# Sbte/RAILS

Hardware: AMD Instinct MI355X
Metric: RAILS iterations/sec (+ A*V SpMM HBM GB/s in roofline), m=1M rows/GPU, k=128, fp64 (higher is better)
Workload: dtype f64

## Files before the change

### include/rails_hip.h

```cpp
#ifndef RAILS_HIP_H
#define RAILS_HIP_H

#include <stddef.h>
#include <stdint.h>

#ifdef __cplusplus
extern "C" {
#endif

#define RAILS_OK 0
#define RAILS_EINVAL -1
#define RAILS_EHIP -2
#define RAILS_ENOMEM -3
#define RAILS_ELAPACK -4
#define RAILS_ECOMM -5
#define RAILS_ENODEV -6

typedef struct rails_ctx rails_ctx;
typedef struct rails_csr rails_csr;
typedef struct rails_panel rails_panel;

const char *rails_last_error(void);
const char *rails_version(void);


int rails_ctx_create(int device, void *stream, rails_ctx **out);
int rails_ctx_destroy(rails_ctx *ctx);
int rails_ctx_sync(rails_ctx *ctx);
void *rails_ctx_stream(rails_ctx *ctx);
int rails_ctx_stats(rails_ctx *ctx, char *buf, int cap);
int rails_ctx_set_meter(rails_ctx *ctx, int on);

int rails_ctx_set_seed(rails_ctx *ctx, uint64_t seed, uint64_t first_stream);
int rails_ctx_rng_state(rails_ctx *ctx, uint64_t *seed, uint64_t *next_stream);

int rails_ctx_set_partition(rails_ctx *ctx, int rank, int nranks, int64_t row0, int64_t m_global);

typedef int (*rails_allreduce_fn)(void *user, double *dev_buf, size_t n, void *stream);
int rails_ctx_set_allreduce(rails_ctx *ctx, rails_allreduce_fn fn, void *user);

#define RAILS_RCCL_ID_BYTES 128
int rails_rccl_unique_id(void *id_out);
int rails_ctx_init_rccl(rails_ctx *ctx, const void *id, int nranks, int rank);
int rails_ctx_set_rccl(rails_ctx *ctx, void *nccl_comm);
int rails_ctx_rccl_size(const rails_ctx *ctx);

typedef int (*rails_halo_fn)(void *user, const double *send_buf, double *recv_buf, int ncols, void *stream);


int rails_csr_create(rails_ctx *ctx, int64_t m_local, int64_t n_cols_ext, const int64_t *rowptr,
                     const int32_t *col, const double *val, rails_csr **out);
typedef int (*rails_apply_fn)(void *user, int trans, const rails_panel *X, int xc0, int nc, rails_panel *Y, int yc0);
int rails_csr_create_callback(rails_ctx *ctx, int64_t m_local, rails_apply_fn fn, void *user, rails_csr **out);
int rails_csr_destroy(rails_csr *A);
int64_t rails_csr_rows(const rails_csr *A);
int64_t rails_csr_nnz(const rails_csr *A);

int rails_csr_set_halo(rails_csr *A, int64_t n_send, const int64_t *send_rows, int64_t n_ghost,
                       rails_halo_fn fn, void *user);

int rails_csr_set_halo_counts(rails_csr *A, int nranks, const int64_t *send_counts, const int64_t *recv_counts);

int rails_spmm(rails_ctx *ctx, rails_csr *A, int trans, const rails_panel *X, int xc0, int nc,
               rails_panel *Y, int yc0);

int rails_csr_set_variant(rails_csr *A, int variant);
int rails_csr_prepare(rails_ctx *ctx, rails_csr *A, int trans, int nc, int *kernel_ready);
int rails_csr_sweep_stats(rails_csr *A, int nc, double *out);
int rails_csr_create_rect(rails_ctx *ctx, int64_t n_rows, int64_t n_cols, const int64_t *rowptr, const int32_t *col, const double *val,
                          rails_csr **out);
const char *rails_csr_last_kernel(const rails_csr *A);

typedef struct rails_sptrsv rails_sptrsv;
int rails_sptrsv_create(rails_ctx *ctx, int64_t n, const int64_t *rowptr, const int32_t *col, const double *val, int lower, int unit_diag,
                        rails_sptrsv **out);
void rails_sptrsv_destroy(rails_sptrsv *T);
int64_t rails_sptrsv_levels(const rails_sptrsv *T);
int rails_sptrsv_solve(rails_ctx *ctx, const rails_sptrsv *T, rails_panel *X, int c0, int nc);
int rails_panel_permute_rows(rails_ctx *ctx, const rails_panel *X, int xc0, int nc, const int32_t *perm_dev, int scatter, rails_panel *Y, int yc0);
int rails_index_upload(rails_ctx *ctx, const int32_t *host, int64_t n, int32_t **out_dev);
void rails_index_free(rails_ctx *ctx, int32_t *dev);

typedef struct rails_lu rails_lu;
int rails_lu_create(rails_ctx *ctx, int64_t n, const int64_t *L_rowptr, const int32_t *L_col, const double *L_val, const int64_t *U_rowptr,
                    const int32_t *U_col, const double *U_val, const int32_t *perm_r, const int32_t *perm_c, const int32_t *rows, int64_t m_sub,
                    rails_lu **out);
void rails_lu_destroy(rails_lu *lu);
int rails_lu_solve(rails_ctx *ctx, rails_lu *lu, int trans, const rails_panel *X, int xc0, int nc, rails_panel *Y, int yc0);
int rails_lu_stats(const rails_lu *lu, int64_t *info, int cap);
int rails_csr_create_lu(rails_ctx *ctx, rails_lu *lu, rails_csr **out);

typedef struct rails_sweep_plan rails_sweep_plan;
int rails_sweep_plan_create(int64_t m, int64_t ncols, const int64_t *rowptr, const int32_t *col, const double *val,
                            const int *params, rails_sweep_plan **out);
int rails_sweep_plan_destroy(rails_sweep_plan *plan);
int rails_sweep_plan_info(const rails_sweep_plan *plan, int64_t *iinfo, double *dinfo);
int rails_sweep_plan_array(const rails_sweep_plan *plan, int which, const void **ptr, int64_t *count);


int rails_panel_create(rails_ctx *ctx, int64_t m_local, int capacity, rails_panel **out);
int rails_panel_destroy(rails_panel *P);
int64_t rails_panel_rows(const rails_panel *P);
int rails_panel_capacity(const rails_panel *P);
int rails_panel_ld(const rails_panel *P);
void *rails_panel_device_ptr(const rails_panel *P);
int rails_panel_reserve(rails_ctx *ctx, rails_panel *P, int capacity);

int rails_panel_upload(rails_ctx *ctx, rails_panel *P, int c0, int nc, const double *host, int64_t ldh);
int rails_panel_download(rails_ctx *ctx, const rails_panel *P, int c0, int nc, double *host, int64_t ldh);

int rails_panel_fill(rails_ctx *ctx, rails_panel *P, int c0, int nc, double value);
int rails_panel_scale(rails_ctx *ctx, rails_panel *P, int c0, int nc, double s);
int rails_panel_copy(rails_ctx *ctx, const rails_panel *X, int xc0, int nc, rails_panel *Y, int yc0);
int rails_panel_axpy(rails_ctx *ctx, double alpha, const rails_panel *X, int xc0, int nc, rails_panel *Y,
                     int yc0);
int rails_panel_random(rails_ctx *ctx, rails_panel *P, int c0, int nc);

int rails_gram(rails_ctx *ctx, const rails_panel *X, int xc0, int a, const rails_panel *Y, int yc0, int b,
               double *C_host, int ldc);

int rails_panel_gemm(rails_ctx *ctx, double alpha, const rails_panel *X, int xc0, int k, const double *C_host,
                     int ldc, int r, double beta, rails_panel *Y, int yc0);

int rails_ctx_enable_library_gemm(rails_ctx *ctx);
int rails_ctx_library_gemm_ready(const rails_ctx *ctx);

int rails_deferred_reserve(rails_ctx *ctx, int nslots, int64_t doubles_per_slot);
int rails_gram_deferred(rails_ctx *ctx, const rails_panel *X, int xc0, int a, const rails_panel *Y, int yc0, int b, int slot);
int rails_panel_gemm_deferred(rails_ctx *ctx, double alpha, const rails_panel *X, int xc0, int k, int slot, int ld, int r, double beta,
                              rails_panel *Y, int yc0);
int rails_chol_inverse_deferred(rails_ctx *ctx, int slot_in, int w, int slot_out);
int rails_update_gram_deferred(rails_ctx *ctx, double alpha, const rails_panel *X, int xc0, int k, const double *C_host, int ldc, int r,
                               rails_panel *Y, int yc0, int r2, int slot);
int rails_deferred_fetch(rails_ctx *ctx, int slot, int64_t n, double *host_out);

int rails_panel_gemm_wide(rails_ctx *ctx, double alpha, const rails_panel *X, int xc0, int k, const double *C_host, int ldc, int r,
                          double beta, rails_panel *Y, int yc0);

int rails_orthogonalize(rails_ctx *ctx, rails_panel *V, int k_old, int w, int method, int *used);
int rails_orthogonalize_deflated(rails_ctx *ctx, rails_panel *V, int k_old, int w, const rails_panel *N, int nc0, int q, int method, int *used);

int rails_resid_lanczos(rails_ctx *ctx, const rails_panel *AV, int avc0, const rails_panel *MV, int mvc0, int k,
                        const double *T_host, int ldt, const rails_panel *B, int bc0, int p, int L,
                        double *H_host, int ldh, int *steps);

int rails_lanczos_start(rails_ctx *ctx, const rails_panel *AV, int avc0, const rails_panel *MV, int mvc0, int k,
                        const rails_panel *B, int bc0, int p, double *sums_host);

int rails_lanczos_vectors(rails_ctx *ctx, const double *S_host, int lds, int w, rails_panel *Out, int oc0);
int rails_lanczos_last_launch(rails_ctx *ctx, int *nch, int *unroll, int *nblocks);
int rails_lanczos_release(rails_ctx *ctx);

int rails_ctx_reserve_staging(rails_ctx *ctx, size_t bytes);
int rails_timer_start(rails_ctx *ctx);
int rails_timer_stop(rails_ctx *ctx, double *ms);


void rails_sb03md(char dico, char job, char fact, char trans, int n, double *A, int lda, double *X, int ldx,
                  double *scale, int *info);
void rails_sb03md_counts(long *smith, long *schur);
void rails_sb03md_adi_counts(long *extended, long *fresh);
void rails_sb03md_set_pause(int calls);
void rails_dsyev(char jobz, char uplo, int n, double *a, int lda, double *w, int *info);
void rails_dsteqr(char compz, int n, double *d, double *e, double *z, int ldz, double *work, int *info);
void rails_dgemm(char transa, char transb, int m, int n, int k, double alpha, const double *A, int lda, const double *B,
                 int ldb, double beta, double *C, int ldc);
void rails_dtrsm(char side, char uplo, char transa, char diag, int m, int n, double alpha, const double *A, int lda, double *B, int ldb);
void rails_dpotrf(char uplo, int n, double *a, int lda, int *info);
void rails_dpstrf(char uplo, int n, double *a, int lda, int *piv, int *rank, double tol, int *info);
void rails_range_basis(int m, int n, double *a, int lda, double tol, double *q, int ldq, int *rank, int *info);
int rails_host_lapack_init(const char *path);
const char *rails_host_lapack_path(void);

#ifdef __cplusplus
}
#endif
#endif
```

### rails_amd/_lib.py

```python
import ctypes as C
import os

_HERE = os.path.dirname(os.path.abspath(__file__))
LIB_PATH = os.path.join(_HERE, "lib", "librails_hip.so")

_dp = C.POINTER(C.c_double)
_ip = C.POINTER(C.c_int)
_i64p = C.POINTER(C.c_int64)
_i32p = C.POINTER(C.c_int32)
_vp = C.c_void_p

ALLREDUCE_FN = C.CFUNCTYPE(C.c_int, C.c_void_p, C.c_void_p, C.c_size_t, C.c_void_p)
HALO_FN = C.CFUNCTYPE(C.c_int, C.c_void_p, C.c_void_p, C.c_void_p, C.c_int, C.c_void_p)
APPLY_FN = C.CFUNCTYPE(C.c_int, C.c_void_p, C.c_int, C.c_void_p, C.c_int, C.c_int, C.c_void_p, C.c_int)

SIGNATURES = {
    "rails_last_error": (C.c_char_p, []),
    "rails_version": (C.c_char_p, []),
    "rails_ctx_create": (C.c_int, [C.c_int, _vp, C.POINTER(_vp)]),
    "rails_ctx_destroy": (C.c_int, [_vp]),
    "rails_ctx_sync": (C.c_int, [_vp]),
    "rails_ctx_stream": (_vp, [_vp]),
    "rails_ctx_set_meter": (C.c_int, [_vp, C.c_int]),
    "rails_ctx_enable_library_gemm": (C.c_int, [_vp]),
    "rails_ctx_library_gemm_ready": (C.c_int, [_vp]),
    "rails_deferred_reserve": (C.c_int, [_vp, C.c_int, C.c_int64]),
    "rails_gram_deferred": (C.c_int, [_vp, _vp, C.c_int, C.c_int, _vp, C.c_int, C.c_int, C.c_int]),
    "rails_update_gram_deferred": (C.c_int, [_vp, C.c_double, _vp, C.c_int, C.c_int, _dp, C.c_int, C.c_int, _vp, C.c_int, C.c_int, C.c_int]),
    "rails_panel_gemm_deferred": (C.c_int, [_vp, C.c_double, _vp, C.c_int, C.c_int, C.c_int, C.c_int, C.c_int, C.c_double, _vp, C.c_int]),
    "rails_chol_inverse_deferred": (C.c_int, [_vp, C.c_int, C.c_int, C.c_int]),
    "rails_deferred_fetch": (C.c_int, [_vp, C.c_int, C.c_int64, _dp]),
    "rails_ctx_stats": (C.c_int, [_vp, C.c_char_p, C.c_int]),
    "rails_ctx_set_seed": (C.c_int, [_vp, C.c_uint64, C.c_uint64]),
    "rails_ctx_rng_state": (C.c_int, [_vp, C.POINTER(C.c_uint64), C.POINTER(C.c_uint64)]),
    "rails_ctx_set_partition": (C.c_int, [_vp, C.c_int, C.c_int, C.c_int64, C.c_int64]),
    "rails_ctx_set_allreduce": (C.c_int, [_vp, ALLREDUCE_FN, _vp]),
    "rails_rccl_unique_id": (C.c_int, [_vp]),
    "rails_ctx_init_rccl": (C.c_int, [_vp, _vp, C.c_int, C.c_int]),
    "rails_ctx_set_rccl": (C.c_int, [_vp, _vp]),
    "rails_ctx_rccl_size": (C.c_int, [_vp]),
    "rails_csr_set_halo_counts": (C.c_int, [_vp, C.c_int, _i64p, _i64p]),
    "rails_csr_create": (C.c_int, [_vp, C.c_int64, C.c_int64, _i64p, _i32p, _dp, C.POINTER(_vp)]),
    "rails_csr_create_rect": (C.c_int, [_vp, C.c_int64, C.c_int64, _i64p, _i32p, _dp, C.POINTER(_vp)]),
    "rails_csr_create_callback": (C.c_int, [_vp, C.c_int64, APPLY_FN, _vp, C.POINTER(_vp)]),
    "rails_csr_destroy": (C.c_int, [_vp]),
    "rails_csr_rows": (C.c_int64, [_vp]),
    "rails_csr_nnz": (C.c_int64, [_vp]),
    "rails_csr_set_halo": (C.c_int, [_vp, C.c_int64, _i64p, C.c_int64, HALO_FN, _vp]),
    "rails_spmm": (C.c_int, [_vp, _vp, C.c_int, _vp, C.c_int, C.c_int, _vp, C.c_int]),
    "rails_csr_set_variant": (C.c_int, [_vp, C.c_int]),
    "rails_csr_sweep_stats": (C.c_int, [_vp, C.c_int, _dp]),
    "rails_csr_prepare": (C.c_int, [_vp, _vp, C.c_int, C.c_int, C.POINTER(C.c_int)]),
    "rails_csr_last_kernel": (C.c_char_p, [_vp]),
    "rails_sweep_plan_create": (C.c_int, [C.c_int64, C.c_int64, _i64p, _i32p, _dp, _ip, C.POINTER(_vp)]),
    "rails_sweep_plan_destroy": (C.c_int, [_vp]),
    "rails_sweep_plan_info": (C.c_int, [_vp, _i64p, _dp]),
    "rails_sweep_plan_array": (C.c_int, [_vp, C.c_int, C.POINTER(_vp), _i64p]),
    "rails_panel_create": (C.c_int, [_vp, C.c_int64, C.c_int, C.POINTER(_vp)]),
    "rails_panel_destroy": (C.c_int, [_vp]),
    "rails_panel_rows": (C.c_int64, [_vp]),
    "rails_panel_capacity": (C.c_int, [_vp]),
    "rails_panel_ld": (C.c_int, [_vp]),
    "rails_panel_device_ptr": (_vp, [_vp]),
    "rails_panel_reserve": (C.c_int, [_vp, _vp, C.c_int]),
    "rails_panel_upload": (C.c_int, [_vp, _vp, C.c_int, C.c_int, _dp, C.c_int64]),
    "rails_panel_download": (C.c_int, [_vp, _vp, C.c_int, C.c_int, _dp, C.c_int64]),
    "rails_panel_fill": (C.c_int, [_vp, _vp, C.c_int, C.c_int, C.c_double]),
    "rails_panel_scale": (C.c_int, [_vp, _vp, C.c_int, C.c_int, C.c_double]),
    "rails_panel_copy": (C.c_int, [_vp, _vp, C.c_int, C.c_int, _vp, C.c_int]),
    "rails_panel_axpy": (C.c_int, [_vp, C.c_double, _vp, C.c_int, C.c_int, _vp, C.c_int]),
    "rails_sptrsv_create": (C.c_int, [_vp, C.c_int64, _i64p, _i32p, _dp, C.c_int, C.c_int, C.POINTER(_vp)]),
    "rails_sptrsv_destroy": (None, [_vp]),
    "rails_sptrsv_levels": (C.c_int64, [_vp]),
    "rails_sptrsv_solve": (C.c_int, [_vp, _vp, _vp, C.c_int, C.c_int]),
    "rails_panel_permute_rows": (C.c_int, [_vp, _vp, C.c_int, C.c_int, _vp, C.c_int, _vp, C.c_int]),
    "rails_index_upload": (C.c_int, [_vp, _i32p, C.c_int64, C.POINTER(_vp)]),
    "rails_index_free": (None, [_vp, _vp]),
    "rails_lu_create": (C.c_int, [_vp, C.c_int64, _i64p, _i32p, _dp, _i64p, _i32p, _dp, _i32p, _i32p, _i32p, C.c_int64, C.POINTER(_vp)]),
    "rails_lu_destroy": (None, [_vp]),
    "rails_lu_solve": (C.c_int, [_vp, _vp, C.c_int, _vp, C.c_int, C.c_int, _vp, C.c_int]),
    "rails_lu_stats": (C.c_int, [_vp, _i64p, C.c_int]),
    "rails_csr_create_lu": (C.c_int, [_vp, _vp, C.POINTER(_vp)]),
    "rails_panel_random": (C.c_int, [_vp, _vp, C.c_int, C.c_int]),
    "rails_gram": (C.c_int, [_vp, _vp, C.c_int, C.c_int, _vp, C.c_int, C.c_int, _dp, C.c_int]),
    "rails_panel_gemm": (C.c_int, [_vp, C.c_double, _vp, C.c_int, C.c_int, _dp, C.c_int, C.c_int, C.c_double, _vp, C.c_int]),
    "rails_panel_gemm_wide": (C.c_int, [_vp, C.c_double, _vp, C.c_int, C.c_int, _dp, C.c_int, C.c_int, C.c_double, _vp, C.c_int]),
    "rails_orthogonalize": (C.c_int, [_vp, _vp, C.c_int, C.c_int, C.c_int, _ip]),
    "rails_orthogonalize_deflated": (C.c_int, [_vp, _vp, C.c_int, C.c_int, _vp, C.c_int, C.c_int, C.c_int, _ip]),
    "rails_resid_lanczos": (C.c_int, [_vp, _vp, C.c_int, _vp, C.c_int, C.c_int, _dp, C.c_int, _vp, C.c_int, C.c_int, C.c_int,
                                      _dp, C.c_int, _ip]),
    "rails_lanczos_start": (C.c_int, [_vp, _vp, C.c_int, _vp, C.c_int, C.c_int, _vp, C.c_int, C.c_int, _dp]),
    "rails_lanczos_vectors": (C.c_int, [_vp, _dp, C.c_int, C.c_int, _vp, C.c_int]),
    "rails_lanczos_last_launch": (C.c_int, [_vp, _ip, _ip, _ip]),
    "rails_lanczos_release": (C.c_int, [_vp]),
    "rails_timer_start": (C.c_int, [_vp]),
    "rails_timer_stop": (C.c_int, [_vp, _dp]),
    "rails_sb03md": (None, [C.c_char, C.c_char, C.c_char, C.c_char, C.c_int, _dp, C.c_int, _dp, C.c_int, _dp, _ip]),
    "rails_dsyev": (None, [C.c_char, C.c_char, C.c_int, _dp, C.c_int, _dp, _ip]),
    "rails_dsteqr": (None, [C.c_char, C.c_int, _dp, _dp, _dp, C.c_int, _dp, _ip]),
    "rails_ctx_reserve_staging": (C.c_int, [_vp, C.c_size_t]),
    "rails_sb03md_set_pause": (None, [C.c_int]),
    "rails_sb03md_counts": (None, [C.POINTER(C.c_long), C.POINTER(C.c_long)]),
    "rails_sb03md_adi_counts": (None, [C.POINTER(C.c_long), C.POINTER(C.c_long)]),
    "rails_dtrsm": (None, [C.c_char, C.c_char, C.c_char, C.c_char, C.c_int, C.c_int, C.c_double, _dp, C.c_int, _dp, C.c_int]),
    "rails_dgemm": (None, [C.c_char, C.c_char, C.c_int, C.c_int, C.c_int, C.c_double, _dp, C.c_int, _dp, C.c_int, C.c_double, _dp, C.c_int]),
    "rails_dpotrf": (None, [C.c_char, C.c_int, _dp, C.c_int, _ip]),
    "rails_dpstrf": (None, [C.c_char, C.c_int, _dp, C.c_int, _ip, _ip, C.c_double, _ip]),
    "rails_range_basis": (None, [C.c_int, C.c_int, _dp, C.c_int, C.c_double, _dp, C.c_int, _ip, _ip]),
    "rails_host_lapack_init": (C.c_int, [C.c_char_p]),
    "rails_host_lapack_path": (C.c_char_p, []),
}

_lib = None


class RailsError(RuntimeError):
    pass


def load():
    global _lib
    if _lib is not None:
        return _lib
    if not os.path.exists(LIB_PATH):
        raise RailsError(
            "rails_amd: %s is missing -- build it with `python -c 'import __graft_entry__ as g; g.build()'` "
            "or `make -C rails_amd/csrc`; there is no CPU fallback" % LIB_PATH)
    lib = C.CDLL(LIB_PATH, mode=C.RTLD_GLOBAL)
    for name, (res, args) in SIGNATURES.items():
        fn = getattr(lib, name)
        fn.restype = res
        fn.argtypes = args
    try:
        from ._solver_sigs import bind as _bind_solver
        _bind_solver(lib)
    except ImportError:
        pass
    from ._solution_sigs import bind as _bind_solution

    _bind_solution(lib)
    _lib = lib
    return lib


def check(rc, what=""):
    if rc != 0:
        msg = load().rails_last_error()
        raise RailsError("%s failed (code %d): %s" % (what or "rails call", rc, msg.decode() if msg else ""))
```

### rails_amd/csrc/host_numerics.cpp

```cpp
#include <dlfcn.h>

#include <algorithm>
#include <atomic>
#include <chrono>
#include <utility>
#include <cmath>
#include <cstdio>
#include <cstdlib>
#include <cstring>
#include <mutex>
#include <string>
#include <vector>

#include "rails_hip.h"

void rails_set_error(const char *fmt, ...);

namespace {

extern "C" {
typedef int (*lp_select2)(const double *, const double *);
typedef void (*lp_dsyev)(const char *, const char *, const int *, double *, const int *, double *, double *, const int *, int *);
typedef void (*lp_dsyevd)(const char *, const char *, const int *, double *, const int *, double *, double *, const int *, int *, const int *, int *);
typedef void (*lp_dsteqr)(const char *, const int *, double *, double *, double *, const int *, double *, int *);
// ... 106 lines not shown
    return true;
}

void gemm(char ta, char tb, int m, int n, int k, const double *A, int lda, const double *B, int ldb, double *C, int ldc)
{
    const double one = 1.0, zero = 0.0;
    g_lp.dgemm(&ta, &tb, &m, &n, &k, &one, A, &lda, B, &ldb, &zero, C, &ldc);
}

}

extern "C" int rails_host_lapack_init(const char *path)
{
    std::lock_guard<std::mutex> lock(g_lp_mutex);
    if (g_lp.handle) return RAILS_OK;
    if (path && *path && try_open(path)) return RAILS_OK;
    if (const char *env = getenv("RAILS_LAPACK_LIB"))
        if (try_open(env)) return RAILS_OK;
    static const char *dirs[] = {"/usr/local/lib/python3.10/dist-packages/scipy.libs", "/usr/lib/python3/dist-packages/scipy.libs",
                                 nullptr};
    for (int i = 0; dirs[i]; ++i) {
        std::string cmd = std::string("ls ") + dirs[i] + "/libscipy_openblas*.so 2>/dev/null";
        if (FILE *f = popen(cmd.c_str(), "r")) {
            char buf[1024];
            std::vector<std::string> found;
            while (fgets(buf, sizeof(buf), f)) {
                std::string s(buf);
                while (!s.empty() && (s.back() == '\n' || s.back() == ' ')) s.pop_back();
                found.push_back(s);
            }
            pclose(f);
            for (auto &s : found)
                if (try_open(s)) return RAILS_OK;
        }
    }
    static const char *cands[] = {"libopenblas.so.0", "libopenblas.so", "liblapack.so.3", "liblapack.so", "/opt/conda/lib/libmkl_rt.so",
                                  "libmkl_rt.so", nullptr};
    for (int i = 0; cands[i]; ++i)
        if (try_open(cands[i])) return RAILS_OK;
    rails_set_error("no host LAPACK found: set RAILS_LAPACK_LIB to a library exporting dsyev_/dgees_/dtrsyl_/dpotrf_/dgemm_");
    return RAILS_ELAPACK;
}

extern "C" const char *rails_host_lapack_path(void) { return g_lp.path.c_str(); }

static bool all_finite(int rows, int cols, const double *a, int lda)
{
    for (int j = 0; j < cols; ++j)
        for (int i = 0; i < rows; ++i)
            if (!std::isfinite(a[i + (size_t)j * lda])) return false;
    return true;
}

extern "C" void rails_dsyev(char jobz, char uplo, int n, double *a, int lda, double *w, int *info)
{
    if (rails_host_lapack_init(nullptr) != RAILS_OK) {
        *info = -100;
        return;
    }
    if (n <= 0) {
        *info = 0;
        return;
    }
    if (!all_finite(n, n, a, lda)) {
        fprintf(stderr, "rails_dsyev: the matrix holds NaN or Inf entries\n");
        *info = n + 1;
        return;
    }
    if (g_lp.dsyevd && n >= 64 && (jobz == 'V' || jobz == 'v')) {
        int lwork = -1, liwork = -1, iq = 0;
        double wq = 0.0;
        g_lp.dsyevd(&jobz, &uplo, &n, a, &lda, w, &wq, &lwork, &iq, &liwork, info);
        if (*info == 0) {
            lwork = (int)wq + 1;
            liwork = iq + 1;
            std::vector<double> work((size_t)lwork);
            std::vector<int> iwork((size_t)liwork);
            g_lp.dsyevd(&jobz, &uplo, &n, a, &lda, w, work.data(), &lwork, iwork.data(), &liwork, info);
            return;
        }
    }
    int lwork = -1;
    double wq = 0.0;
    g_lp.dsyev(&jobz, &uplo, &n, a, &lda, w, &wq, &lwork, info);
    if (*info) return;
    lwork = (int)wq;
    std::vector<double> work((size_t)std::max(1, lwork));
    g_lp.dsyev(&jobz, &uplo, &n, a, &lda, w, work.data(), &lwork, info);
}

extern "C" void rails_dsteqr(char compz, int n, double *d, double *e, double *z, int ldz, double *work, int *info)
{
    if (rails_host_lapack_init(nullptr) != RAILS_OK) {
        *info = -100;
        return;
    }
    g_lp.dsteqr(&compz, &n, d, e, z, &ldz, work, info);
}

extern "C" void rails_dtrsm(char side, char uplo, char transa, char diag, int m, int n, double alpha, const double *A, int lda, double *B, int ldb)
{
    if (m <= 0 || n <= 0) return;
    const char *force_loops = getenv("RAILS_DTRSM_LOOPS");
    if (!(force_loops && atoi(force_loops) != 0) && rails_host_lapack_init(nullptr) == RAILS_OK && g_lp.dtrsm) {
        g_lp.dtrsm(&side, &uplo, &transa, &diag, &m, &n, &alpha, A, &lda, B, &ldb);
        return;
    }
    const bool left = side == 'L' || side == 'l', upper = uplo == 'U' || uplo == 'u', trans = !(transa == 'N' || transa == 'n'),
               unit = diag == 'U' || diag == 'u';
    const int na = left ? m : n;
    auto a = [&](int i, int j) { return trans ? A[j + (size_t)i * lda] : A[i + (size_t)j * lda]; };
    const bool op_upper = upper != trans;
    for (int j = 0; j < n; ++j)
        for (int i = 0; i < m; ++i) B[i + (size_t)j * ldb] *= alpha;
    if (left) {
        for (int j = 0; j < n; ++j) {
            double *b = B + (size_t)j * ldb;
            if (op_upper)
                for (int i = na - 1; i >= 0; --i) {
                    double s = b[i];
                    for (int l = i + 1; l < na; ++l) s -= a(i, l) * b[l];
                    b[i] = unit ? s : s / a(i, i);
                }
            else
                for (int i = 0; i < na; ++i) {
                    double s = b[i];
                    for (int l = 0; l < i; ++l) s -= a(i, l) * b[l];
                    b[i] = unit ? s : s / a(i, i);
                }
        }
    } else {
        for (int i = 0; i < m; ++i) {
            if (op_upper)
                for (int j = 0; j < na; ++j) {
                    double s = B[i + (size_t)j * ldb];
                    for (int l = 0; l < j; ++l) s -= B[i + (size_t)l * ldb] * a(l, j);
                    B[i + (size_t)j * ldb] = unit ? s : s / a(j, j);
                }
            else
                for (int j = na - 1; j >= 0; --j) {
                    double s = B[i + (size_t)j * ldb];
                    for (int l = j + 1; l < na; ++l) s -= B[i + (size_t)l * ldb] * a(l, j);
                    B[i + (size_t)j * ldb] = unit ? s : s / a(j, j);
                }
        }
    }
}

extern "C" void rails_dgemm(char ta, char tb, int m, int n, int k, double alpha, const double *A, int lda, const double *B, int ldb,
                            double beta, double *C, int ldc)
{
    if (rails_host_lapack_init(nullptr) != RAILS_OK) return;
    g_lp.dgemm(&ta, &tb, &m, &n, &k, &alpha, A, &lda, B, &ldb, &beta, C, &ldc);
}

extern "C" void rails_dpotrf(char uplo, int n, double *a, int lda, int *info)
{
    if (rails_host_lapack_init(nullptr) != RAILS_OK) {
        *info = -100;
        return;
    }
    g_lp.dpotrf(&uplo, &n, a, &lda, info);
}

extern "C" void rails_dpstrf(char uplo, int n, double *a, int lda, int *piv, int *rank, double tol, int *info)
{
    if (rails_host_lapack_init(nullptr) != RAILS_OK) {
        *info = -100;
        return;
    }
    if (g_lp.dpstrf) {
        std::vector<double> work((size_t)2 * (n > 0 ? n : 1));
        g_lp.dpstrf(&uplo, &n, a, &lda, piv, rank, &tol, work.data(), info);
        for (int i = 0; i < n; ++i) piv[i] -= 1;
        return;
    }
    *info = 0;
    if (uplo != 'U' && uplo != 'u') {
        *info = -1;
        return;
    }
    for (int i = 0; i < n; ++i) piv[i] = i;
    int r = 0;
    for (; r < n; ++r) {
        int q = r;
        for (int j = r + 1; j < n; ++j)
            if (a[j + (size_t)j * lda] > a[q + (size_t)q * lda]) q = j;
        if (!(a[q + (size_t)q * lda] > tol)) break;
        if (q != r) {
            std::swap(piv[r], piv[q]);
            std::swap(a[r + (size_t)r * lda], a[q + (size_t)q * lda]);
            for (int i = 0; i < r; ++i) std::swap(a[i + (size_t)r * lda], a[i + (size_t)q * lda]);
            for (int j = q + 1; j < n; ++j) std::swap(a[r + (size_t)j * lda], a[q + (size_t)j * lda]);
            for (int i = r + 1; i < q; ++i) std::swap(a[r + (size_t)i * lda], a[i + (size_t)q * lda]);
        }
        double d = std::sqrt(a[r + (size_t)r * lda]);
        a[r + (size_t)r * lda] = d;
        for (int j = r + 1; j < n; ++j) a[r + (size_t)j * lda] /= d;
        for (int j = r + 1; j < n; ++j) {
            double f = a[r + (size_t)j * lda];
            for (int i = r + 1; i <= j; ++i) a[i + (size_t)j * lda] -= a[r + (size_t)i * lda] * f;
        }
    }
    *rank = r;
    *info = r < n ? 1 : 0;
}

extern "C" void rails_range_basis(int m, int n, double *a, int lda, double tol, double *q, int ldq, int *rank, int *info)
{
    *rank = 0;
    if (rails_host_lapack_init(nullptr) != RAILS_OK || !g_lp.dgeqp3 || !g_lp.dorgqr) {
        *info = -100;
        return;
    }
    if (m <= 0 || n <= 0) {
        *info = 0;
        return;
    }
    const int kmin = m < n ? m : n;
    std::vector<int> jpvt((size_t)n, 0);
    std::vector<double> tau((size_t)kmin);
    double wq = 0.0;
    int lwork = -1;
    g_lp.dgeqp3(&m, &n, a, &lda, jpvt.data(), tau.data(), &wq, &lwork, info);
    if (*info != 0) return;
    lwork = (int)wq + 1;
    std::vector<double> work((size_t)lwork);
    g_lp.dgeqp3(&m, &n, a, &lda, jpvt.data(), tau.data(), work.data(), &lwork, info);
    if (*info != 0) return;
    const double r11 = std::fabs(a[0]);
    int r = 0;
    while (r < kmin && std::fabs(a[r + (size_t)r * lda]) > tol * r11 && r11 > 0.0) ++r;
    *rank = r;
    if (r == 0) return;
    for (int j = 0; j < r; ++j)
        for (int i = 0; i < m; ++i) q[i + (size_t)j * ldq] = a[i + (size_t)j * lda];
    lwork = -1;
    g_lp.dorgqr(&m, &r, &r, q, &ldq, tau.data(), &wq, &lwork, info);
    if (*info != 0) return;
    lwork = (int)wq + 1;
    work.resize((size_t)lwork);
    g_lp.dorgqr(&m, &r, &r, q, &ldq, tau.data(), work.data(), &lwork, info);
}

static int &sb03md_smith_pause()
{
    static thread_local int pause = 0;
    return pause;
}
static int &sb03md_factored_pause()
{
    static thread_local int pause = 0;
    return pause;
}
extern "C" void rails_sb03md_set_pause(int calls) { sb03md_smith_pause() = sb03md_factored_pause() = calls > 0 ? calls : 0; }
static std::atomic<long> g_sb03md_smith{0}, g_sb03md_schur{0};
extern "C" void rails_sb03md_counts(long *smith, long *schur)
{
    if (smith) *smith = g_sb03md_smith.load();
    if (schur) *schur = g_sb03md_schur.load();
}

static bool smith_lyapunov(bool tr, int n, const double *A, int lda, double *X, int ldx)
{
    if (!g_lp.dgetrf || !g_lp.dgetrs) return false;
    const size_t nn = (size_t)n * n;
    std::vector<double> M(nn), S(nn), Ak(nn), Y(nn), T1(nn), T2(nn), C(nn);
    double trace = 0.0;
    for (int j = 0; j < n; ++j) {
        for (int i = 0; i < n; ++i) {
            M[i + (size_t)j * n] = tr ? A[i + (size_t)j * lda] : A[j + (size_t)i * lda];
            C[i + (size_t)j * n] = 0.5 * (X[i + (size_t)j * ldx] + X[j + (size_t)i * ldx]);
        }
        trace += A[j + (size_t)j * lda];
    }
    const double p = -trace / n;
    if (!(p > 0.0) || !std::isfinite(p)) return false;
    S = M;
    for (int j = 0; j < n; ++j) S[j + (size_t)j * n] -= p;
    std::vector<int> ipiv(n);
    int info = 0;
    g_lp.dgetrf(&n, &n, S.data(), &n, ipiv.data(), &info);
    if (info != 0) return false;
    std::fill(Ak.begin(), Ak.end(), 0.0);
    for (int j = 0; j < n; ++j) Ak[j + (size_t)j * n] = 1.0;
    const char N = 'N';
    g_lp.dgetrs(&N, &n, &n, S.data(), &n, ipiv.data(), Ak.data(), &n, &info);
    if (info != 0) return false;
    gemm('N', 'N', n, n, n, Ak.data(), n, C.data(), n, T1.data(), n);
    gemm('N', 'T', n, n, n, T1.data(), n, Ak.data(), n, Y.data(), n);
    for (size_t q = 0; q < nn; ++q) Y[q] *= -2.0 * p;
    for (size_t q = 0; q < nn; ++q) Ak[q] *= 2.0 * p;
    for (int j = 0; j < n; ++j) Ak[j + (size_t)j * n] += 1.0;
    auto fro = [&](std::vector<double> const &Z) {
        double s2 = 0.0;
        for (size_t q = 0; q < nn; ++q) s2 += Z[q] * Z[q];
        return std::sqrt(s2);
    };
    bool converged = false;
    for (int k = 0; k < 10; ++k) {
        gemm('N', 'N', n, n, n, Ak.data(), n, Y.data(), n, T1.data(), n);
        gemm('N', 'T', n, n, n, T1.data(), n, Ak.data(), n, T2.data(), n);
        const double inc = fro(T2), ny = fro(Y);
        if (!std::isfinite(inc) || inc > 10.0 * ny) return false;
        for (size_t q = 0; q < nn; ++q) Y[q] += T2[q];
        if (inc <= 1e-8 * ny) {
// ... 538 lines not shown
```

### rails_amd/include/rails/SubspaceSolverOps.hpp

```cpp
#ifndef RAILS_SUBSPACESOLVEROPS_HPP
#define RAILS_SUBSPACESOLVEROPS_HPP

#include "rails/LyapunovSolver.hpp"
#include "rails/SubspaceWrappers.hpp"

namespace rails
{

template <>
struct SolverOps<SubspaceOperator, SubspaceMultiVector, HostDenseMatrix> {
    typedef Solver<SubspaceOperator, SubspaceMultiVector, HostDenseMatrix> SolverT;
    struct State {
    };
    struct Lanczos {
        HostDenseMatrix eigenvalues;
        SubspaceMultiVector eigenvectors;
        void append_to(SubspaceMultiVector &V, std::vector<int> const &indices, int count) const
        {
            for (int i = 0; i < count; i++) V.push_back(eigenvectors.view(indices[i]));
        }
    };
    static SubspaceMultiVector apply_append(SubspaceOperator const &A, SubspaceMultiVector const &W, SubspaceMultiVector &AV)
    {
        SubspaceMultiVector AW = A * W;
        AV.push_back(AW);
        return AW;
    }
    static int lanczos(SolverT &solver, State &, SubspaceMultiVector const &AV, SubspaceMultiVector const &MV, HostDenseMatrix const &T,
                       HostDenseMatrix const &, SubspaceMultiVector const &, int max_iter, Lanczos &out)
    {
        HostDenseMatrix H(max_iter + 1, max_iter + 1);
        out.eigenvalues = HostDenseMatrix(max_iter, 1);
        return solver.resid_lanczos(AV, MV, T, H, out.eigenvectors, out.eigenvalues, max_iter);
    }
    static void multiply_inplace(SubspaceMultiVector &V, HostDenseMatrix const &X)
    {
        V.view(0, X.N() - 1) = V * X;
        V.resize(X.N());
        V.discard_unused_columns();
    }
    static void on_restart(State &, HostDenseMatrix const &, SubspaceMultiVector &V, SubspaceMultiVector &)
    {
        if (V.basis()) V.basis()->compress();
    }
};

typedef Solver<SubspaceOperator, SubspaceMultiVector, HostDenseMatrix> SubspaceSolver;

}

#endif
```

### rails_amd/include/rails/SubspaceWrappers.hpp

```cpp
#ifndef RAILS_SUBSPACEWRAPPERS_HPP
#define RAILS_SUBSPACEWRAPPERS_HPP

#include <algorithm>
#include <atomic>
#include <chrono>
#include <cmath>
#include <cstdlib>
#include <cstring>
#include <iostream>
#include <memory>
#include <vector>

#include "rails/HipWrappers.hpp"

namespace rails
{

struct CoefStore {
    std::vector<double> c;
    int ld = 0, ncap = 0;
    bool in_basis = true;
    CoefStore(int ld_, int ncap_, bool in_basis_) : c((size_t)std::max(ld_, 1) * std::max(ncap_, 1), 0.0), ld(ld_), ncap(std::max(ncap_, 1)), in_basis(in_basis_) {}
    double *col(int j) { return c.data() + (size_t)j * ld; }
    const double *col(int j) const { return c.data() + (size_t)j * ld; }
// ... 565 lines not shown
            for (int j = 0; j < dim; ++j)
                for (int i = 0; i < dim; ++i) orth = std::max(orth, std::fabs(PP[i + (size_t)j * dim] - (i == j ? 1.0 : 0.0)));
            if (trace) std::cerr << "absorb (overlapped) verified: dim " << d0 << " -> " << dim << ": |P'P - I| = " << orth << std::endl;
            verify_orth = std::max(verify_orth, orth);
        }
        return !failed;
    }

private:
    bool fail(const char *what = nullptr)
    {
        if (what) std::cerr << "rails_amd: SubspaceBasis: " << what << std::endl;
        failed = true;
        return false;
    }

    static void upper_inverse(std::vector<double> const &R, int r, std::vector<double> &Rinv)
    {
        for (int j = 0; j < r; ++j) {
            Rinv[j + (size_t)j * r] = 1.0 / R[j + (size_t)j * r];
            for (int i = j - 1; i >= 0; --i) {
                double s = 0.0;
                for (int l = i + 1; l <= j; ++l) s += R[i + (size_t)l * r] * Rinv[l + (size_t)j * r];
                Rinv[i + (size_t)j * r] = -s / R[i + (size_t)i * r];
            }
        }
    }

    bool absorb_one_by_one(int w, double *coef, std::vector<int> const &keep, std::vector<double> const &colscale)
    {
        n_single++;
        const int ld = row_cap;
        rails_panel *pp = P.panel();
        const int base = dim;
        int accepted = 0;
        for (int idx = 0; idx < (int)keep.size(); ++idx) {
            const int j = keep[idx];
            const int src = base + j, dst = base + accepted;
            if (src != dst && !hip_ok(rails_panel_copy(ctx, pp, src, 1, pp, dst), "rails_panel_copy")) return fail();
            double g0 = 0.0, g = 0.0;
            if (!hip_ok(rails_gram(ctx, pp, dst, 1, pp, dst, 1, &g0, 1), "rails_gram")) return fail();
            for (int round = 0; round < 2 && accepted > 0; ++round) {
                const int nb = base + accepted;
                std::vector<double> c(nb);
                if (!hip_ok(rails_gram(ctx, pp, 0, nb, pp, dst, 1, c.data(), nb), "rails_gram")) return fail();
                if (!hip_ok(rails_panel_gemm(ctx, -1.0, pp, 0, nb, c.data(), nb, 1, 1.0, pp, dst), "rails_panel_gemm")) return fail();
                for (int a = 0; a < nb; ++a) coef[a + (size_t)j * ld] += colscale[j] * c[a];
            }
            if (!hip_ok(rails_gram(ctx, pp, dst, 1, pp, dst, 1, &g, 1), "rails_gram")) return fail();
            if (!(g > 1e-24 * g0) || !(g > 0.0)) {
                n_dropped++;
                if (trace) std::cerr << "absorb one by one: column " << j << " dropped: " << g << " left of " << g0 << " (scale " << colscale[j] << ")" << std::endl;
                continue;
            }
            const double nrm = std::sqrt(g);
            if (!hip_ok(rails_panel_scale(ctx, pp, dst, 1, 1.0 / nrm), "rails_panel_scale")) return fail();
            double last = nrm;
            if (g < 1e-8 * g0 && base + accepted > 0) {
                const int nb = base + accepted;
                std::vector<double> c(nb);
                double n2 = 0.0;
                if (!hip_ok(rails_gram(ctx, pp, 0, nb, pp, dst, 1, c.data(), nb), "rails_gram")) return fail();
                if (!hip_ok(rails_panel_gemm(ctx, -1.0, pp, 0, nb, c.data(), nb, 1, 1.0, pp, dst), "rails_panel_gemm")) return fail();
                if (!hip_ok(rails_gram(ctx, pp, dst, 1, pp, dst, 1, &n2, 1), "rails_gram")) return fail();
                for (int a = 0; a < nb; ++a) coef[a + (size_t)j * ld] += colscale[j] * nrm * c[a];
                if (!(n2 > 0.25)) {
                    n_dropped++;
                    if (trace) std::cerr << "absorb one by one: column " << j << " dropped after the check against the whole basis: " << n2 << " of its unit length left (it was " << colscale[j] * nrm << " long)" << std::endl;
                    continue;
                }
                if (!hip_ok(rails_panel_scale(ctx, pp, dst, 1, 1.0 / std::sqrt(n2)), "rails_panel_scale")) return fail();
                last = nrm * std::sqrt(n2);
            }
            coef[(base + accepted) + (size_t)j * ld] = colscale[j] * last;
            if (trace) std::cerr << "absorb one by one: column " << j << " -> basis column " << base + accepted << ": " << g << " left of " << g0 << " (scale " << colscale[j] << ")" << std::endl;
            if (verify && trace && base + accepted > 0) {
                std::vector<double> c(base + accepted);
                rails_gram(ctx, pp, 0, base + accepted, pp, dst, 1, c.data(), base + accepted);
                double e = 0.0;
                int at = -1;
                for (int a = 0; a < base + accepted; ++a)
                    if (std::fabs(c[a]) > e) { e = std::fabs(c[a]); at = a; }
                std::cerr << "    against the basis so far: " << e << " at column " << at << std::endl;
            }
            accepted++;
        }
        dim = base + accepted;
        P.resize(dim);
        return true;
    }
};

class SubspaceOperator;

class SubspaceMultiVector
{
    friend class SubspaceOperator;
    std::shared_ptr<SubspaceBasis> basis_;
    std::shared_ptr<CoefStore> store_;
    int c0_ = 0, n_ = -1;
    int orthogonalized_ = 0;
    bool is_view_ = false, transpose_ = false;

    int rows() const { return !store_ ? 0 : (store_->in_basis ? basis_->dim : store_->ld); }
    double *cptr(int j = 0) const { return store_->col(c0_ + j); }
    int ld() const { return store_->ld; }
    bool in_basis() const { return !store_ || store_->in_basis; }

    void ensure_cols(int n)
    {
        if (!store_) return;
        if (c0_ + n <= store_->ncap) return;
        int ncap = c0_ + n;
        store_->c.resize((size_t)store_->ld * ncap, 0.0);
        store_->ncap = ncap;
    }

public:
    SubspaceMultiVector() {}

    SubspaceMultiVector(std::shared_ptr<SubspaceBasis> const &b, int n) : basis_(b), store_(b->new_store(std::max(n, 1), true)), n_(n) {}

    static SubspaceMultiVector Plain(std::shared_ptr<SubspaceBasis> const &b, int rows, int n)
    {
        SubspaceMultiVector out;
        out.basis_ = b;
        out.store_ = b->new_store(std::max(n, 1), false, rows);
        out.n_ = n;
        return out;
    }

    SubspaceMultiVector(SubspaceMultiVector const &o)
        : basis_(o.basis_), c0_(0), n_(o.n_), orthogonalized_(o.orthogonalized_), is_view_(false), transpose_(o.transpose_)
    {
        if (o.store_) {
            int cap = std::max(o.store_->ncap - o.c0_, 1);
            store_ = basis_->new_store(cap, o.store_->in_basis, o.store_->ld);
            for (int j = 0; j < std::max(o.n_, 0); ++j) memcpy(store_->col(j), o.cptr(j), sizeof(double) * o.rows());
        }
    }
    SubspaceMultiVector(SubspaceMultiVector &&o) = default;

    SubspaceMultiVector(SubspaceMultiVector const &o, int n)
        : basis_(o.basis_), n_(n)
    {
        if (o.store_) store_ = basis_->new_store(std::max(n, 1), o.store_->in_basis, o.store_->ld);
    }

    virtual ~SubspaceMultiVector() {}

    std::shared_ptr<SubspaceBasis> const &basis() const { return basis_; }
    const double *coefficients() const { return cptr(); }
    int coefficient_ld() const { return ld(); }
    int coefficient_rows() const { return rows(); }

    SubspaceMultiVector &operator=(SubspaceMultiVector const &o)
    {
        if (!is_view_) {
            basis_ = o.basis_;
            store_ = o.store_;
            c0_ = o.c0_;
            n_ = o.n_;
            orthogonalized_ = o.orthogonalized_;
            transpose_ = o.transpose_;
            return *this;
        }
        int cols = std::min(n_, o.n_);
        for (int j = 0; j < cols; ++j) memcpy(cptr(j), o.cptr(j), sizeof(double) * rows());
        return *this;
    }

    SubspaceMultiVector &operator=(double v)
    {
        orthogonalized_ = 0;
        if (!store_ || n_ <= 0) return *this;
        if (!in_basis() || v == 0.0) {
            for (int j = 0; j < n_; ++j) std::fill_n(cptr(j), in_basis() ? ld() : rows(), v);
            return *this;
        }
        SubspaceBasis &b = *basis_;
        int t0 = b.tail(1);
        b.P.resize(t0 + 1);
        if (!hip_ok(rails_panel_fill(b.ctx, b.P.panel(), t0, 1, v), "rails_panel_fill")) b.failed = true;
        b.P.resize(t0);
        std::fill_n(cptr(0), ld(), 0.0);
        b.absorb_tail(1, cptr(0));
        for (int j = 1; j < n_; ++j) memcpy(cptr(j), cptr(0), sizeof(double) * ld());
        return *this;
    }

    SubspaceMultiVector &operator*=(double s)
    {
        for (int j = 0; j < n_; ++j) {
            double *c = cptr(j);
            for (int i = 0, r = rows(); i < r; ++i) c[i] *= s;
        }
        orthogonalized_ = 0;
        return *this;
    }
    SubspaceMultiVector &operator/=(double s) { return *this *= 1.0 / s; }

    SubspaceMultiVector &axpy(double a, SubspaceMultiVector const &o)
    {
        int cols = std::min(n_, o.n_);
        for (int j = 0; j < cols; ++j) {
            double *c = cptr(j);
            const double *x = o.cptr(j);
            for (int i = 0, r = rows(); i < r; ++i) c[i] += a * x[i];
        }
        orthogonalized_ = 0;
        return *this;
    }
    SubspaceMultiVector &operator+=(SubspaceMultiVector const &o) { return axpy(1.0, o); }
    SubspaceMultiVector &operator-=(SubspaceMultiVector const &o) { return axpy(-1.0, o); }
    SubspaceMultiVector operator+(SubspaceMultiVector const &o) const
    {
        SubspaceMultiVector out(*this);
        out += o;
        return out;
    }

    int M() const { return transpose_ ? n_ : (in_basis() ? (basis_ ? (int)basis_->m_global : -1) : store_->ld); }
    int N() const { return transpose_ ? (in_basis() ? (basis_ ? (int)basis_->m_global : -1) : store_->ld) : n_; }

    void resize(int n)
    {
        orthogonalized_ = std::min(orthogonalized_, n);
        ensure_cols(n);
        n_ = n;
    }

    void discard_unused_columns()
    {
        if (!store_ || is_view_) return;
        for (int j = c0_ + std::max(n_, 0); j < store_->ncap; ++j) std::fill_n(store_->col(j), store_->ld, 0.0);
    }

    SubspaceMultiVector view(int a = -1, int b = -1) const
    {
        SubspaceMultiVector out;
        out.basis_ = basis_;
        out.store_ = store_;
        out.transpose_ = transpose_;
        out.is_view_ = true;
        int num = 1;
        if (b > 0 && a >= 0)
            num = b - a + 1;
        else if (a < 0) {
            a = 0;
            num = n_;
        }
        out.c0_ = c0_ + a;
        out.n_ = num;
        return out;
    }

    SubspaceMultiVector copy() const { return SubspaceMultiVector(*this); }

    void push_back(SubspaceMultiVector const &o)
    {
        if (!store_) {
            basis_ = o.basis_;
            store_ = basis_->new_store(std::max(o.n_, 1), o.store_->in_basis, o.store_->ld);
            n_ = 0;
        }
        int n = n_, on = o.n_;
        resize(n + on);
        for (int j = 0; j < on; ++j) memcpy(cptr(n + j), o.cptr(j), sizeof(double) * rows());
    }

    void random()
    {
        if (!in_basis() || n_ <= 0) {
            if (!in_basis()) std::cerr << "rails_amd: random() on a plain replicated object is not supported" << std::endl;
            return;
        }
        SubspaceBasis &b = *basis_;
        orthogonalized_ = 0;
        if (b.cached_valid) {
            b.cached_valid = false;
            if (n_ == 1) {
                memcpy(cptr(0), b.cached_random->col(0), sizeof(double) * ld());
                std::fill_n(b.cached_random->col(0), b.cached_random->ld, 0.0);
                return;
            }
            std::cerr << "rails_amd: a prefetched random vector is discarded (random() on " << n_ << " columns)" << std::endl;
        }
        for (int j0 = 0; j0 < n_; j0 += 64) {
            int w = std::min(64, n_ - j0);
            int t0 = b.tail(w);
            b.P.resize(t0 + w);
            if (!hip_ok(rails_panel_random(b.ctx, b.P.panel(), t0, w), "rails_panel_random")) b.failed = true;
            b.P.resize(t0);
            for (int j = 0; j < w; ++j) std::fill_n(cptr(j0 + j), ld(), 0.0);
            b.absorb_tail(w, cptr(j0));
        }
        orthogonalized_ = 0;
    }

    SubspaceMultiVector transpose() const
    {
        SubspaceMultiVector out = view();
        out.is_view_ = false;
        out.transpose_ = !transpose_;
        out.orthogonalized_ = orthogonalized_;
        return out;
// ... 210 lines not shown
```

Before: 226.5.

## Run residual Lanczos in subspace coordinates with a native SIMD host kernel

Adds a host routine that runs the residual Lanczos iteration directly on the subspace coefficient arrays (AV, V, B, T), using vectorised dot products and linear combinations with an AVX2/FMA dispatch. The solver's lanczos hook calls it when all operands share the same subspace basis, and otherwise falls back to the generic resid_lanczos. This aims to remove per-step overhead from generic operator and multivector dispatch and full Hessenberg orthogonalisation. The trade-off is that it uses only three-term recurrence without full reorthogonalisation, which may change numerics and convergence behaviour.

```diff
diff --git a/include/rails_hip.h b/include/rails_hip.h
--- a/include/rails_hip.h
+++ b/include/rails_hip.h
@@ -165,6 +165,9 @@
 void rails_dsteqr(char compz, int n, double *d, double *e, double *z, int ldz, double *work, int *info);
 void rails_dgemm(char transa, char transb, int m, int n, int k, double alpha, const double *A, int lda, const double *B,
                  int ldb, double beta, double *C, int ldc);
+int rails_coord_resid_lanczos(int dim, int k, int p, const double *AV, int ldav, const double *V, int ldv, const double *B, int ldb,
+                              const double *T, int ldt, int max_steps, double *alpha, double *beta, double *Q, int ldq, int *steps);
+long rails_coord_resid_lanczos_calls(void);
 void rails_dtrsm(char side, char uplo, char transa, char diag, int m, int n, double alpha, const double *A, int lda, double *B, int ldb);
 void rails_dpotrf(char uplo, int n, double *a, int lda, int *info);
 void rails_dpstrf(char uplo, int n, double *a, int lda, int *piv, int *rank, double tol, int *info);
diff --git a/rails_amd/_lib.py b/rails_amd/_lib.py
--- a/rails_amd/_lib.py
+++ b/rails_amd/_lib.py
@@ -104,6 +104,9 @@
     "rails_sb03md_adi_counts": (None, [C.POINTER(C.c_long), C.POINTER(C.c_long)]),
     "rails_dtrsm": (None, [C.c_char, C.c_char, C.c_char, C.c_char, C.c_int, C.c_int, C.c_double, _dp, C.c_int, _dp, C.c_int]),
     "rails_dgemm": (None, [C.c_char, C.c_char, C.c_int, C.c_int, C.c_int, C.c_double, _dp, C.c_int, _dp, C.c_int, C.c_double, _dp, C.c_int]),
+    "rails_coord_resid_lanczos": (C.c_int, [C.c_int, C.c_int, C.c_int, _dp, C.c_int, _dp, C.c_int, _dp, C.c_int, _dp, C.c_int, C.c_int, _dp, _dp, _dp,
+                                            C.c_int, _ip]),
+    "rails_coord_resid_lanczos_calls": (C.c_long, []),
     "rails_dpotrf": (None, [C.c_char, C.c_int, _dp, C.c_int, _ip]),
     "rails_dpstrf": (None, [C.c_char, C.c_int, _dp, C.c_int, _ip, _ip, C.c_double, _ip]),
     "rails_range_basis": (None, [C.c_int, C.c_int, _dp, C.c_int, C.c_double, _dp, C.c_int, _ip, _ip]),
diff --git a/rails_amd/csrc/host_numerics.cpp b/rails_amd/csrc/host_numerics.cpp
--- a/rails_amd/csrc/host_numerics.cpp
+++ b/rails_amd/csrc/host_numerics.cpp
@@ -282,6 +282,163 @@
 {
     if (rails_host_lapack_init(nullptr) != RAILS_OK) return;
     g_lp.dgemm(&ta, &tb, &m, &n, &k, &alpha, A, &lda, B, &ldb, &beta, C, &ldc);
+}
+
+namespace {
+
+typedef double lz_v4 __attribute__((vector_size(32), aligned(8), may_alias));
+
+#define LZ_INLINE static inline __attribute__((always_inline))
+
+LZ_INLINE lz_v4 lz_load(const double *p) { return *reinterpret_cast<const lz_v4 *>(p); }
+LZ_INLINE void lz_store(double *p, lz_v4 v) { *reinterpret_cast<lz_v4 *>(p) = v; }
+LZ_INLINE double lz_hsum(lz_v4 v) { return (v[0] + v[1]) + (v[2] + v[3]); }
+
+LZ_INLINE double lz_dot(int n, const double *x, const double *y)
+{
+    lz_v4 s0 = {0, 0, 0, 0}, s1 = {0, 0, 0, 0};
+    int i = 0;
+    for (; i + 8 <= n; i += 8) {
+        s0 += lz_load(x + i) * lz_load(y + i);
+        s1 += lz_load(x + i + 4) * lz_load(y + i + 4);
+    }
+    double s = lz_hsum(s0 + s1);
+    for (; i < n; ++i) s += x[i] * y[i];
+    return s;
+}
+
+LZ_INLINE void lz_dots(int rows, int n, const double *X, int ldx, const double *q, double *y)
+{
+    int j = 0;
+    for (; j + 4 <= n; j += 4) {
+        const double *x0 = X + (size_t)j * ldx, *x1 = x0 + ldx, *x2 = x1 + ldx, *x3 = x2 + ldx;
+        lz_v4 a0 = {0, 0, 0, 0}, a1 = a0, a2 = a0, a3 = a0, b0 = a0, b1 = a0, b2 = a0, b3 = a0;
+        int i = 0;
+        for (; i + 8 <= rows; i += 8) {
+            const lz_v4 qa = lz_load(q + i), qb = lz_load(q + i + 4);
+            a0 += lz_load(x0 + i) * qa;
+            b0 += lz_load(x0 + i + 4) * qb;
+            a1 += lz_load(x1 + i) * qa;
+            b1 += lz_load(x1 + i + 4) * qb;
+            a2 += lz_load(x2 + i) * qa;
+            b2 += lz_load(x2 + i + 4) * qb;
+            a3 += lz_load(x3 + i) * qa;
+            b3 += lz_load(x3 + i + 4) * qb;
+        }
+        double s0 = lz_hsum(a0 + b0), s1 = lz_hsum(a1 + b1), s2 = lz_hsum(a2 + b2), s3 = lz_hsum(a3 + b3);
+        for (; i < rows; ++i) {
+            s0 += x0[i] * q[i];
+            s1 += x1[i] * q[i];
+            s2 += x2[i] * q[i];
+            s3 += x3[i] * q[i];
+        }
+        y[j] = s0;
+        y[j + 1] = s1;
+        y[j + 2] = s2;
+        y[j + 3] = s3;
+    }
+    for (; j < n; ++j) y[j] = lz_dot(rows, X + (size_t)j * ldx, q);
+}
+
+LZ_INLINE void lz_combine(int rows, int n, const double *X, int ldx, const double *c, double *out)
+{
+    for (int i = 0; i < rows; ++i) out[i] = 0.0;
+    int j = 0;
+    for (; j + 4 <= n; j += 4) {
+        const double *x0 = X + (size_t)j * ldx, *x1 = x0 + ldx, *x2 = x1 + ldx, *x3 = x2 + ldx;
+        const double c0 = c[j], c1 = c[j + 1], c2 = c[j + 2], c3 = c[j + 3];
+        const lz_v4 v0 = {c0, c0, c0, c0}, v1 = {c1, c1, c1, c1}, v2 = {c2, c2, c2, c2}, v3 = {c3, c3, c3, c3};
+        int i = 0;
+        for (; i + 4 <= rows; i += 4)
+            lz_store(out + i, lz_load(out + i) + ((lz_load(x0 + i) * v0 + lz_load(x1 + i) * v1) + (lz_load(x2 + i) * v2 + lz_load(x3 + i) * v3)));
+        for (; i < rows; ++i) out[i] += (x0[i] * c0 + x1[i] * c1) + (x2[i] * c2 + x3[i] * c3);
+    }
+    for (; j < n; ++j) {
+        const double *x = X + (size_t)j * ldx;
+        const double cj = c[j];
+        for (int i = 0; i < rows; ++i) out[i] += x[i] * cj;
+    }
+}
+
+struct LzArgs {
+    int dim, k, p;
+    const double *AV, *V, *B, *T;
+    int ldav, ldv, ldb, ldt, max_steps;
+    double *alpha, *beta, *Q;
+    int ldq;
+    double *work;
+};
+
+LZ_INLINE int lz_run(LzArgs const &a)
+{
+    const int dim = a.dim, k = a.k, p = a.p;
+    double *y = a.work, *ty = y + 2 * k, *yb = ty + 2 * k, *tb = yb + p, *ta = tb + dim, *tv = ta + dim;
+    int steps = 0;
+    double off = 0.0;
+    while (steps < a.max_steps) {
+        const int j = steps++;
+        const double *q = a.Q + (size_t)j * a.ldq;
+        double *r = a.Q + (size_t)(j + 1) * a.ldq;
+        lz_dots(dim, k, a.V, a.ldv, q, y);
+        lz_dots(dim, k, a.AV, a.ldav, q, y + k);
+        lz_dots(dim, p, a.B, a.ldb, q, yb);
+        if (k > 0) {
+            const double one = 1.0, zero = 0.0;
+            const int two = 2;
+            g_lp.dgemm("N", "N", &k, &two, &k, &one, a.T, &a.ldt, y, &k, &zero, ty, &k);
+        }
+        lz_combine(dim, p, a.B, a.ldb, yb, tb);
+        lz_combine(dim, k, a.AV, a.ldav, ty, ta);
+        lz_combine(dim, k, a.V, a.ldv, ty + k, tv);
+        for (int i = 0; i < dim; ++i) r[i] = (tb[i] + ta[i]) + tv[i];
+        const double diag = lz_dot(dim, r, q);
+        a.alpha[j] = diag;
+        for (int i = 0; i < dim; ++i) r[i] -= diag * q[i];
+        if (j > 0) {
+            const double *qp = a.Q + (size_t)(j - 1) * a.ldq;
+            for (int i = 0; i < dim; ++i) r[i] -= off * qp[i];
+        }
+        off = std::sqrt(std::fabs(lz_dot(dim, r, r)));
+        if (off < 1e-14) break;
+        a.beta[j] = off;
+        const double inv = 1.0 / off;
+        for (int i = 0; i < dim; ++i) r[i] *= inv;
+    }
+    return steps;
+}
+
+int lz_run_baseline(LzArgs const &a) { return lz_run(a); }
+#if defined(__x86_64__)
+__attribute__((target("avx2,fma"))) int lz_run_avx2(LzArgs const &a) { return lz_run(a); }
+#endif
+
+#undef LZ_INLINE
+
+}
+
+static std::atomic<long> g_coord_lanczos_calls{0};
+extern "C" long rails_coord_resid_lanczos_calls(void) { return g_coord_lanczos_calls.load(); }
+
+extern "C" int rails_coord_resid_lanczos(int dim, int k, int p, const double *AV, int ldav, const double *V, int ldv, const double *B, int ldb,
+                                         const double *T, int ldt, int max_steps, double *alpha, double *beta, double *Q, int ldq, int *steps_out)
+{
+    if (dim < 1 || k < 0 || p < 0 || max_steps < 1 || !alpha || !beta || !Q || ldq < dim || !steps_out || (k > 0 && (!AV || !V || !T)) ||
+        (p > 0 && !B) || (k > 0 && (ldav < dim || ldv < dim || ldt < k)) || (p > 0 && ldb < dim)) {
+        rails_set_error("rails_coord_resid_lanczos: bad argument (dim %d, k %d, p %d, steps %d)", dim, k, p, max_steps);
+        return RAILS_EINVAL;
+    }
+    if (rails_host_lapack_init(nullptr) != RAILS_OK) return RAILS_ELAPACK;
+    g_coord_lanczos_calls++;
+    std::vector<double> work((size_t)4 * k + p + (size_t)3 * dim + 8, 0.0);
+    for (int j = 0; j < max_steps; ++j) alpha[j] = beta[j] = 0.0;
+    LzArgs a{dim, k, p, AV, V, B, T, ldav, ldv, ldb, std::max(ldt, 1), max_steps, alpha, beta, Q, ldq, work.data()};
+#if defined(__x86_64__)
+    static const bool wide = __builtin_cpu_supports("avx2") && __builtin_cpu_supports("fma") && !(getenv("RAILS_COORD_LANCZOS_BASELINE") && atoi(getenv("RAILS_COORD_LANCZOS_BASELINE")) != 0);
+    *steps_out = wide ? lz_run_avx2(a) : lz_run_baseline(a);
+#else
+    *steps_out = lz_run_baseline(a);
+#endif
+    return RAILS_OK;
 }
 
 extern "C" void rails_dpotrf(char uplo, int n, double *a, int lda, int *info)
diff --git a/rails_amd/include/rails/SubspaceSolverOps.hpp b/rails_amd/include/rails/SubspaceSolverOps.hpp
--- a/rails_amd/include/rails/SubspaceSolverOps.hpp
+++ b/rails_amd/include/rails/SubspaceSolverOps.hpp
@@ -29,9 +29,44 @@
     static int lanczos(SolverT &solver, State &, SubspaceMultiVector const &AV, SubspaceMultiVector const &MV, HostDenseMatrix const &T,
                        HostDenseMatrix const &, SubspaceMultiVector const &, int max_iter, Lanczos &out)
     {
-        HostDenseMatrix H(max_iter + 1, max_iter + 1);
         out.eigenvalues = HostDenseMatrix(max_iter, 1);
-        return solver.resid_lanczos(AV, MV, T, H, out.eigenvectors, out.eigenvalues, max_iter);
+        const bool native = !(getenv("RAILS_COORD_LANCZOS") && atoi(getenv("RAILS_COORD_LANCZOS")) == 0);
+        const int k = AV.N();
+        bool in_basis = native && max_iter >= 1 && !solver.B().given_as_operator() && AV.basis() && AV.basis()->dim >= 1 && !AV.replicated() &&
+                        !MV.replicated() && MV.basis() == AV.basis() && MV.N() == k && k >= 0 && T.M() == k && T.N() == k && !T.transposed();
+        if (in_basis) {
+            SubspaceMultiVector const &Bp = solver.B().panel();
+            in_basis = Bp.basis() == AV.basis() && !Bp.replicated() && Bp.N() >= 0;
+        }
+        if (!in_basis) {
+            HostDenseMatrix H(max_iter + 1, max_iter + 1);
+            return solver.resid_lanczos(AV, MV, T, H, out.eigenvectors, out.eigenvalues, max_iter);
+        }
+        SubspaceMultiVector const &B = solver.B().panel();
+        SubspaceMultiVector Q(MV, max_iter + 1);
+        Q.resize(1);
+        Q.random();
+        Q.view(0) /= Q.norm();
+        Q.resize(max_iter + 1);
+        const int dim = AV.coefficient_rows(), p = B.N();
+        std::vector<double> alpha(max_iter), beta(max_iter);
+        int steps = 0;
+        if (rails_coord_resid_lanczos(dim, k, p, AV.coefficients(), AV.coefficient_ld(), MV.coefficients(), MV.coefficient_ld(), B.coefficients(),
+                                      B.coefficient_ld(), (double *)T, T.raw_ld(), max_iter, alpha.data(), beta.data(), Q.mutable_coefficients(),
+                                      Q.coefficient_ld(), &steps) != RAILS_OK) {
+            std::cerr << "rails_amd: rails_coord_resid_lanczos failed: " << rails_last_error() << std::endl;
+            return -1;
+        }
+        HostDenseMatrix H(steps, steps);
+        for (int j = 0; j < steps; ++j) {
+            H(j, j) = alpha[j];
+            if (j + 1 < steps) H(j + 1, j) = H(j, j + 1) = beta[j];
+        }
+        Q.resize(steps);
+        HostDenseMatrix ritz(steps, steps);
+        H.eigs(ritz, out.eigenvalues);
+        out.eigenvectors = Q * ritz;
+        return 0;
     }
     static void multiply_inplace(SubspaceMultiVector &V, HostDenseMatrix const &X)
     {
diff --git a/rails_amd/include/rails/SubspaceWrappers.hpp b/rails_amd/include/rails/SubspaceWrappers.hpp
--- a/rails_amd/include/rails/SubspaceWrappers.hpp
+++ b/rails_amd/include/rails/SubspaceWrappers.hpp
@@ -741,6 +741,11 @@
     std::shared_ptr<SubspaceBasis> const &basis() const { return basis_; }
     const double *coefficients() const { return cptr(); }
     int coefficient_ld() const { return ld(); }
+    double *mutable_coefficients()
+    {
+        orthogonalized_ = 0;
+        return cptr();
+    }
     int coefficient_rows() const { return rows(); }
 
     SubspaceMultiVector &operator=(SubspaceMultiVector const &o)
```

Result: no change. 225.7 (median of 3 runs) (-0.3%).
